# anyboby/Constrained-Model-Based-Policy-Optimization

Hardware: AMD Instinct MI355X
Metric: imagined env-steps/sec (ensemble rollout) + CPO update ms (higher is better)
Workload: dtype f32; 1 GPU; AntSafe-v2 imagined rollout: E=7 x (37->512->512->60) swish ensemble, 5 elites, 3+3 critics 128x128, tanh policy 128x128, B=100000 branches/GPU, maxroll 35 (34 steps), fixed-horizon mode, reset->sample*->finish_all_paths->get(); rollout_mode=schedule, branches_per_gpu=100000, branches_total=100000, horizon=34, task=AntSafe-v2

## Files before the change

constrained-model-based-policy-optimization_amd/csrc/fakeenv_post.hip:

```cpp
#include "common.h"

#include <math.h>

#include <type_traits>

namespace {

typedef float f32x2 __attribute__((ext_vector_type(2)));

constexpr int kThreads = 256;
constexpr int kRows = 8;
constexpr int kEMaxRt = 8;
constexpr int kEMax = kEMaxRt;

struct PostArgs {
  int task, ensemble, obs_dim, act_dim, out_dim;
  int learned_cost;
  const float *mean, *var;
  int ld_rows;
  const float *obs, *act;
  const int32_t *elite, *row_idx, *n_rows_dev;
  int n_rows;
  float *next_obs, *rew;
  uint8_t *term;
// ... 7 lines not shown
  const float *xi;
};
struct PostArgsRulesNoise : PostArgsRules {
  const float *xi;
};
template <bool RULES, bool NOISE>
using PostArgsBase = std::conditional_t<NOISE, std::conditional_t<RULES, PostArgsRulesNoise, PostArgsNoise>,
                                        std::conditional_t<RULES, PostArgsRules, PostArgs>>;
template <bool RULES, bool NOISE>
struct PostArgsDis : PostArgsBase<RULES, NOISE> {
  float kappa_rew, kappa_cost;
  float *rew_var, *cost_var;
};
template <bool RULES, bool NOISE, bool DIS = false>
using PostArgsT = std::conditional_t<DIS, PostArgsDis<RULES, NOISE>, PostArgsBase<RULES, NOISE>>;

__device__ __forceinline__ float clip_np(float x, float lo, float hi) { return x < lo ? lo : (x > hi ? hi : x); }

#define POST_WAVES 5
template <int EC, bool RULES = false, bool NOISE = false, bool DIS = false>
__global__ __launch_bounds__(kThreads) __attribute__((amdgpu_waves_per_eu(POST_WAVES, POST_WAVES))) void fakeenv_post_kernel(const PostArgsT<RULES, NOISE, DIS> p) {
  extern __shared__ float sm[];
  const int D = p.obs_dim;
  float *s_dkl = sm;
  float *s_var = s_dkl + kRows * D;
  float *s_next = s_var + kRows * D;
  int *s_row = reinterpret_cast<int *>(s_next + kRows * D);

  const int tid = threadIdx.x;
  const int n_rows = p.n_rows_dev ? *p.n_rows_dev : p.n_rows;
  const int row0 = blockIdx.x * kRows;
  if (row0 >= n_rows) return;
  if (tid < kRows) {
    const int r = row0 + tid;
    s_row[tid] = (r < n_rows) ? (p.row_idx ? p.row_idx[r] : r) : -1;
  }
  __syncthreads();

  const int E = EC > 0 ? EC : p.ensemble;
  constexpr int kEMax = EC > 0 ? EC : ::kEMaxRt;
  const size_t mstride = (size_t)p.ld_rows * p.out_dim;
  for (int i = tid; i < kRows * D; i += kThreads) {
    const int b = i / D, d = i - b * D;
    const int r = s_row[b];
    if (r < 0) continue;
    float mu[kEMax], ls[kEMax], vr[kEMax];
    bool fast = EC > 0;
    const size_t base = (size_t)r * p.out_dim + d;
    float v0s[kEMax];
#pragma unroll
// ... 95 lines not shown
              const float q = __fmul_rn(num, rden[c]);
              float pre = __fmul_rn(0.5f, __fsub_rn(q, 1.0f));
              pre = __fsub_rn(__fadd_rn(pre, ls[c]), ls[a]);
              pre = clip_np(pre, 0.0f, 1e10f);
              acc = __fadd_rn(acc, pre);
            }
          }
          if (!isfinite(vr[a]) || !isfinite(mu[a])) acc = __fadd_rn(acc, __builtin_nanf(""));
        }
      }
    }
    s_dkl[i] = acc / ((float)(E * (E - 1)) + 1e-10f);
    const float nx = __fadd_rn(mean_me, obs_rd);
    s_next[i] = nx;
    p.next_obs[(size_t)r * D + d] = nx;
    if (p.ep_var) p.ep_var[(size_t)r * D + d] = s_var[i];
  }
  __syncthreads();

  if (tid < 8 * kRows) {
    const int rw = tid >> 3, k = tid & 7;
    const int r = s_row[rw];
    const float *nx = s_next + rw * D;
    [[maybe_unused]] float xr = 0.0f, xc = 0.0f;
    [[maybe_unused]] int me_k = 0;
    if constexpr (DIS) {
      if (r >= 0) {
        me_k = p.elite[r];
        if (k < E) {
          const size_t o = k * mstride + (size_t)r * p.out_dim + D;
// ... 99 lines not shown
      const bool notdone = __fmul_rn(gate, zrot) >= -0.7f;
      done = notdone ? 0 : 1;
      const float obj = (fabsf(nx[D - 1]) > 3.2f) ? 1.0f : 0.0f;
      cost = fminf(fmaxf((float)done + obj, 0.0f), 1.0f);
    } else if (p.task == CMBPO_TASK_HCS) {
      const float xdist = __fmul_rn(nx[D - 1], 10.0f);
      cost = (fabsf(xdist) < 2.0f) ? 1.0f : 0.0f;
    }
    if constexpr (DIS) {
      if (p.learned_cost) cost = p.kappa_cost > 0.0f ? __fadd_rn(cost_me, __fmul_rn(p.kappa_cost, sqrtf(cost_var))) : cost_me;
    } else {
      if (p.learned_cost) cost = p.mean[me * mstride + (size_t)r * p.out_dim + D + 1];
    }
    p.term[r] = done;
    p.cost[r] = cost;
  }
}

template <bool RULES, bool NOISE, bool DIS = false>
void launch_post(int ensemble, dim3 grid, size_t lds, hipStream_t stream, const PostArgsT<RULES, NOISE, DIS> &a) {
  if (ensemble == 7) hipLaunchKernelGGL((fakeenv_post_kernel<7, RULES, NOISE, DIS>), grid, dim3(kThreads), lds, stream, a);
  else if (ensemble == 5) hipLaunchKernelGGL((fakeenv_post_kernel<5, RULES, NOISE, DIS>), grid, dim3(kThreads), lds, stream, a);
  else hipLaunchKernelGGL((fakeenv_post_kernel<0, RULES, NOISE, DIS>), grid, dim3(kThreads), lds, stream, a);
}

struct DisExtra {
  float kappa_rew, kappa_cost;
  float *rew_var, *cost_var;
};
template <bool RULES, bool NOISE>
void launch_post_dis(int ensemble, dim3 grid, size_t lds, hipStream_t stream, const PostArgsBase<RULES, NOISE> &a, const DisExtra &dis) {
  PostArgsDis<RULES, NOISE> ad{};
  static_cast<PostArgsBase<RULES, NOISE> &>(ad) = a;
  ad.kappa_rew = dis.kappa_rew; ad.kappa_cost = dis.kappa_cost; ad.rew_var = dis.rew_var; ad.cost_var = dis.cost_var;
  launch_post<RULES, NOISE, true>(ensemble, grid, lds, stream, ad);
}

int post_impl(const char *who, int task, int ensemble, int obs_dim, int act_dim, const float *d_mean, const float *d_var, int ld_rows,
              const float *d_obs, const float *d_act, const int32_t *d_elite, const int32_t *d_row_idx, const int32_t *d_n_rows,
              int n_rows, float *d_next_obs, float *d_rew, uint8_t *d_term, float *d_cost, float *d_dkl_path, float *d_ep_var_mean,
              float *d_ep_var, const float *d_xi, void *stream, const DisExtra *dis = nullptr) {
  const int learned_cost = (task & CMBPO_TASK_LEARNED_COST) ? 1 : 0;
  const int task_arg = task;
  task &= ~CMBPO_TASK_LEARNED_COST;
  const bool user = task >= CMBPO_TASK_USER_BASE && task < CMBPO_TASK_USER_BASE + CMBPO_TASK_USER_SLOTS;
  CMBPO_REQUIRE((task >= CMBPO_TASK_DEFAULT && task <= CMBPO_TASK_ANTSAFE) || user, "%s: bad task %d", who, task_arg);
  CMBPO_REQUIRE(ensemble >= 2 && ensemble <= kEMax, "%s: ensemble %d not in [2, %d]", who, ensemble, kEMax);
  CMBPO_REQUIRE(obs_dim >= 1 && obs_dim <= 512 && act_dim >= 0, "%s: bad dims", who);
  if (task == CMBPO_TASK_ANTSAFE)
    CMBPO_REQUIRE(obs_dim >= 5, "%s: AntSafe rules need obs_dim >= 5", who);
  PostArgsRules ar{};
  if (user)
    if (int rc = cmbpo_internal_task_rules_resolve(who, task_arg, obs_dim, act_dim, d_act != nullptr, &ar.rules)) return rc;
  CMBPO_REQUIRE(d_mean && d_var && d_obs && d_elite && d_next_obs && d_rew && d_term && d_cost &&
                    d_dkl_path && d_ep_var_mean,
                "%s: NULL buffer", who);
// ... 12 lines not shown
  a.out_dim = obs_dim + 1 + learned_cost;
  a.learned_cost = learned_cost;
  a.mean = d_mean; a.var = d_var; a.ld_rows = ld_rows; a.obs = d_obs; a.act = d_act;
  a.elite = d_elite; a.row_idx = d_row_idx; a.n_rows_dev = d_n_rows; a.n_rows = n_rows;
  a.next_obs = d_next_obs; a.rew = d_rew; a.term = d_term; a.cost = d_cost;
  a.dkl_path = d_dkl_path; a.ep_var_mean = d_ep_var_mean; a.ep_var = d_ep_var;
  const size_t lds = (size_t)3 * kRows * obs_dim * sizeof(float) + kRows * sizeof(int);
  const dim3 grid(cmbpo_ceil_div(n_rows, kRows));
  hipStream_t s = (hipStream_t)stream;
  if (user) static_cast<PostArgs &>(ar) = a;
  if (d_xi != nullptr) {
    if (user) {
      PostArgsRulesNoise an{};
      static_cast<PostArgsRules &>(an) = ar;
      an.xi = d_xi;
      if (dis) launch_post_dis<true, true>(ensemble, grid, lds, s, an, *dis);
      else launch_post<true, true>(ensemble, grid, lds, s, an);
    } else {
      PostArgsNoise an{};
      static_cast<PostArgs &>(an) = a;
      an.xi = d_xi;
      if (dis) launch_post_dis<false, true>(ensemble, grid, lds, s, an, *dis);
      else launch_post<false, true>(ensemble, grid, lds, s, an);
    }
  } else if (dis) {
    if (user) launch_post_dis<true, false>(ensemble, grid, lds, s, ar, *dis);
    else launch_post_dis<false, false>(ensemble, grid, lds, s, a, *dis);
  } else if (user) launch_post<true, false>(ensemble, grid, lds, s, ar);
  else launch_post<false, false>(ensemble, grid, lds, s, a);
  CMBPO_HIP_CHECK(hipGetLastError());
  return CMBPO_OK;
}

}

extern "C" int cmbpo_fakeenv_post(int task, int ensemble, int obs_dim, int act_dim,
                                  const float *d_mean, const float *d_var, int ld_rows,
                                  const float *d_obs, const float *d_act, const int32_t *d_elite,
                                  const int32_t *d_row_idx, const int32_t *d_n_rows, int n_rows,
                                  float *d_next_obs, float *d_rew, uint8_t *d_term, float *d_cost,
                                  float *d_dkl_path, float *d_ep_var_mean, float *d_ep_var,
                                  void *stream) {
  return post_impl("cmbpo_fakeenv_post", task, ensemble, obs_dim, act_dim, d_mean, d_var, ld_rows, d_obs, d_act, d_elite, d_row_idx,
                   d_n_rows, n_rows, d_next_obs, d_rew, d_term, d_cost, d_dkl_path, d_ep_var_mean, d_ep_var, nullptr, stream);
// ... 14 lines not shown
}

extern "C" int cmbpo_fakeenv_post_disagreement(int task, int ensemble, int obs_dim, int act_dim,
                                               const float *d_mean, const float *d_var, int ld_rows,
                                               const float *d_obs, const float *d_act, const int32_t *d_elite,
                                               const int32_t *d_row_idx, const int32_t *d_n_rows, int n_rows,
                                               float *d_next_obs, float *d_rew, uint8_t *d_term, float *d_cost,
                                               float *d_dkl_path, float *d_ep_var_mean, float *d_ep_var,
                                               const float *d_xi, float kappa_rew, float kappa_cost,
                                               float *d_rew_var, float *d_cost_var, void *stream) {
  const DisExtra dis{kappa_rew, kappa_cost, d_rew_var, d_cost_var};
  return post_impl("cmbpo_fakeenv_post_disagreement", task, ensemble, obs_dim, act_dim, d_mean, d_var, ld_rows, d_obs, d_act, d_elite,
                   d_row_idx, d_n_rows, n_rows, d_next_obs, d_rew, d_term, d_cost, d_dkl_path, d_ep_var_mean, d_ep_var, d_xi, stream,
                   &dis);
}
```

constrained-model-based-policy-optimization_amd/csrc/rollout_internal.h:

```cpp
#pragma once
#include "common.h"

int cmbpo_internal_book_post_mirror(const cmbpo_rollout_t *r, int n_alive, uint32_t *d_host_out, uint32_t seq, int spec, int min_alive,
                                    double stop_total, void *stream);
int cmbpo_internal_scalars_mirror(const cmbpo_rollout_t *r, uint32_t *d_host_out, uint32_t seq, void *stream);
int cmbpo_internal_book_pre(const cmbpo_rollout_t *r, int n_alive, int spec, int with_vec, void *stream);
int cmbpo_internal_store_nostats(const cmbpo_rollout_t *r, void *stream);
int cmbpo_internal_finish_post_fold(const cmbpo_rollout_t *r, void *stream);
int cmbpo_internal_spec_words(const cmbpo_rollout_t *r, int begin, void *stream);
int cmbpo_internal_disagreement_lookup(const cmbpo_rollout_t *r, cmbpo_disagreement_t *out);
```

constrained-model-based-policy-optimization_amd/csrc/rollout_state.hip:

```cpp
#include "common.h"
#include "rollout_internal.h"
#include <type_traits>

#include <math.h>

#include <mutex>
#include <unordered_map>

namespace {

constexpr int kScanThreads = 1024;

__device__ __forceinline__ int wave_incl_scan(int v, int lane) {
#pragma unroll
  for (int o = 1; o < 64; o <<= 1) {
    const int t = __shfl_up(v, o, 64);
    if (lane >= o) v += t;
  }
  return v;
}

__device__ __forceinline__ int block_excl_scan(int v, int *sm, int *total) {
  const int lane = threadIdx.x & 63, w = threadIdx.x >> 6, nw = (blockDim.x + 63) >> 6;
  const int inc = wave_incl_scan(v, lane);
// ... 232 lines not shown
    }
    const float cdelta = __fsub_rn(__fadd_rn(c, __fmul_rn(cg32, cvnext)), cv);
    y = __dadd_rn(delta, __dmul_rn(gl, y));
    cy = __dadd_rn((double)cdelta, __dmul_rn(cgl, cy));
    const float adv = (float)y, cadv = (float)cy;
    r.adv_buf[o] = adv;
    r.ret_buf[o] = __fadd_rn(adv, v);
    r.cadv_buf[o] = cadv;
    r.cret_buf[o] = __fadd_rn(cadv, cv);
    vnext = v;
    cvnext = cv;
  }
  r.alive[b] = 0;
}

__device__ __forceinline__ void store_stats_body(const cmbpo_rollout_t &r, const cmbpo_disagreement_t &dg);
__global__ __launch_bounds__(256) void finish_kernel(const cmbpo_rollout_t r, int mode, int fold_stats, const cmbpo_iv_gae_t iv,
                                                  const cmbpo_disagreement_t dg) {
  if (fold_stats && blockIdx.x == 0) store_stats_body(r, dg);
  const int i = blockIdx.x * blockDim.x + threadIdx.x;
  const int n = r.iscal[CMBPO_I_N_ALIVE];
  if (i >= n) return;
  const int b = r.alive_idx[i];
  float lv, lcv;
  bool zero_boot = false;
  if (mode == 0) {
    const uint8_t code = r.fin_code[b];
    if (!code) return;
    lv = r.v_t[b];
    lcv = r.vc_t[b];
    if (code == 2) {
      lv = 0.0f;
      zero_boot = true;
    }
// ... 86 lines not shown
  float *vdst[4] = {r.obs_buf, r.act_buf, r.mu_buf, r.ls_buf};
  const int vdim[4] = {D, A, A, A};
#pragma unroll
  for (int f = 0; f < 4; ++f) {
    const int dim = vdim[f];
    const float inv = 1.0f / (float)dim;
    for (int e = tid; e < rows_here * dim; e += 256) {
      const int k = (int)(((float)e + 0.5f) * inv);
      const int d = e - k * dim;
      const int b = s_slot[k];
      if (b >= 0) vdst[f][((size_t)r.ptr * B + b) * dim + d] = vsrc[f][(size_t)b * dim + d];
    }
  }
}

__device__ __forceinline__ void store_stats_body(const cmbpo_rollout_t &r, const cmbpo_disagreement_t &dg) {
  __shared__ double sm_d[16];
  const int n = r.iscal[CMBPO_I_N_ALIVE];
  const int n_wg = (n + kStoreRows - 1) / kStoreRows;
  double t[8] = {0, 0, 0, 0, 0, 0, 0, 0};
  for (int w = threadIdx.x; w < n_wg; w += 256) {
    const double *src = r.store_part + (size_t)w * 8;
#pragma unroll
    for (int k = 0; k < 6; ++k) t[k] += src[k];
    t[6] = fmax(t[6], src[6]);
    t[7] = fmax(t[7], src[7]);
  }
  double s[8];
#pragma unroll
  for (int k = 0; k < 6; ++k) s[k] = block_sum(t[k], sm_d);
  s[6] = block_max(t[6], sm_d);
  s[7] = block_max(t[7], sm_d);
  if (threadIdx.x == 0 && s[0] > 0.0) {
    const double cnt = s[0];
    const double dkl_mean = r.dscal[CMBPO_D_DKL_SUM_T] / (double)n;
    r.iscal[CMBPO_I_N_STORED] += (int)cnt;
    r.iscal[CMBPO_I_SIZE] += (int)cnt;
    r.dscal[CMBPO_D_TOTAL_SAMPLES] += cnt;
    r.dscal[CMBPO_D_TOTAL_COST] += s[1];
    r.dscal[CMBPO_D_TOTAL_REW] += s[2];
    r.dscal[CMBPO_D_SUM_PATH_RET] += s[2];
// ... 8 lines not shown
  if (dg.part != nullptr) {
    double u0 = 0.0, u1 = 0.0;
    for (int w = threadIdx.x; w < n_wg; w += 256) {
      u0 += dg.part[2 * (size_t)w];
      u1 += dg.part[2 * (size_t)w + 1];
    }
    u0 = block_sum(u0, sm_d);
    u1 = block_sum(u1, sm_d);
    if (threadIdx.x == 0 && s[0] > 0.0) {
      r.dscal[CMBPO_D_TOTAL_REW_VAR] += u0;
      r.dscal[CMBPO_D_TOTAL_COST_VAR] += u1;
    }
  }
}

__global__ __launch_bounds__(256) void store_stats_kernel(const cmbpo_rollout_t r, const cmbpo_disagreement_t dg) { store_stats_body(r, dg); }

constexpr int kBookMax = 1024;

__global__ __launch_bounds__(kScanThreads) void book_pre_kernel(const cmbpo_rollout_t r, int spec, const cmbpo_iv_gae_t iv,
                                                             const cmbpo_disagreement_t dg) {
  __shared__ int sm_i[17];
  __shared__ double sm_d[16];
  __shared__ double sm_m[8 * 16];
  __shared__ int s_unc;
  const int tid = threadIdx.x;
  if (spec && r.iscal[CMBPO_I_HALT]) return;
  const int n = r.iscal[CMBPO_I_N_ALIVE];
  {
    double c = 0.0, d = 0.0;
    for (int i = tid; i < n; i += kScanThreads) {
// ... 785 lines not shown
  CMBPO_REQUIRE(r->cur_obs && r->act_t && r->logp_t && r->mu_t && r->ls_t && r->v_t && r->vc_t && r->rew_t && r->cost_t && r->dkl_t &&
                    r->epv_t && r->obs_buf && r->act_buf && r->mu_buf && r->ls_buf && r->rew_buf && r->val_buf && r->cost_buf &&
                    r->cval_buf && r->logp_buf && r->store_part,
                "cmbpo_rollout_store: NULL array");
  hipLaunchKernelGGL(store_kernel, dim3(cmbpo_ceil_div(r->B, kStoreRows)), dim3(256), 0, (hipStream_t)stream, *r, iv_lookup(r),
                     dg_lookup(r));
  CMBPO_HIP_CHECK(hipGetLastError());
  return CMBPO_OK;
}
int cmbpo_internal_finish_post_fold(const cmbpo_rollout_t *r, void *stream) {
  if (int rc = check_rollout(r, "cmbpo_rollout_finish")) return rc;
  CMBPO_REQUIRE(r->v_n && r->vc_n && r->term_t && r->rew_buf && r->val_buf && r->cost_buf && r->cval_buf && r->adv_buf && r->ret_buf &&
                    r->cadv_buf && r->cret_buf && r->store_part,
                "cmbpo_rollout_finish (POST): NULL array");
  hipLaunchKernelGGL(finish_kernel, dim3(cmbpo_ceil_div(r->B, 256)), dim3(256), 0, (hipStream_t)stream, *r, 1, 1, iv_lookup(r), dg_lookup(r));
  CMBPO_HIP_CHECK(hipGetLastError());
  return CMBPO_OK;
}

extern "C" int cmbpo_rollout_book_pre_max_rows(void) { return kBookMax; }

extern "C" int cmbpo_rollout_book_pre(const cmbpo_rollout_t *r, int n_alive, void *stream) {
  if (int rc = check_rollout(r, "cmbpo_rollout_book_pre")) return rc;
  CMBPO_REQUIRE(n_alive >= 0 && n_alive <= kBookMax, "cmbpo_rollout_book_pre: %d alive rows, at most %d", n_alive, kBookMax);
  CMBPO_REQUIRE(!r->use_host_budget, "cmbpo_rollout_book_pre: the cross-shard budget exchange uses the separate kernels");
  CMBPO_REQUIRE(r->ptr < r->T, "cmbpo_rollout_book_pre: buffer full (ptr %d == T)", r->ptr);
  CMBPO_REQUIRE(r->dkl_t && r->dkl_acc && r->cur_obs && r->act_t && r->logp_t && r->mu_t && r->ls_t && r->v_t && r->vc_t &&
                    r->rew_t && r->cost_t && r->epv_t,
                "cmbpo_rollout_book_pre: NULL step array");
  CMBPO_REQUIRE(r->obs_buf && r->act_buf && r->mu_buf && r->ls_buf && r->rew_buf && r->val_buf && r->cost_buf && r->cval_buf &&
// ... 200 lines not shown
```

constrained-model-based-policy-optimization_amd/csrc/rollout_step.hip:

```cpp
#include "common.h"
#include "ens_mlp_internal.h"
#include "rollout_internal.h"

#include <string.h>
#include <time.h>

#include <atomic>
#include <mutex>

struct Ahead {
  bool on = false;
  int min_alive = 0;
  double stop_total = 0.0;
};

static int step_impl(const cmbpo_rollout_t *r, int n_alive, cmbpo_mlp_t *policy, cmbpo_mlp_t *model, cmbpo_mlp_t *v,
                     cmbpo_mlp_t *vc, int task, int ensemble, const float *d_eps, const int32_t *d_elite, float *d_mean,
                     float *d_var, bool policy_ready, const float *d_eps_next, bool *next_ready, uint32_t *d_mirror, uint32_t seq,
                     const Ahead &ahead, const float *d_xi, void *stream) {
  CMBPO_REQUIRE(r && policy && model && v && vc && d_eps && d_elite && d_mean && d_var, "cmbpo_rollout_step: NULL argument");
  CMBPO_REQUIRE(n_alive >= 1 && n_alive <= r->B, "cmbpo_rollout_step: n_alive %d not in [1, B=%d]", n_alive, r->B);
  CMBPO_REQUIRE(model->out_dim == r->obs_dim + 1 + ((task & CMBPO_TASK_LEARNED_COST) ? 1 : 0),
                "cmbpo_rollout_step: model out_dim %d does not match obs_dim %d + 1 (+ 1 with CMBPO_TASK_LEARNED_COST), task 0x%x",
                model->out_dim, r->obs_dim, task);
  if ((task & ~CMBPO_TASK_LEARNED_COST) >= CMBPO_TASK_USER_BASE)
    if (int rc0 = cmbpo_internal_task_rules_resolve("cmbpo_rollout_step", task, r->obs_dim, r->act_dim, r->act_t != nullptr, nullptr)) return rc0;
  auto w = [](const float *p) { return const_cast<float *>(p); };
  int rc;
  *next_ready = false;
  const int32_t *d_n = ahead.on ? r->iscal + CMBPO_I_N_EFF : nullptr;
  if (ahead.on)
    CMBPO_REQUIRE(n_alive <= cmbpo_rollout_book_pre_max_rows() && !r->use_host_budget && d_mirror && cmbpo_critic_pair_supported(v, vc),
                  "cmbpo_rollout_run: look-ahead needs the small-batch step");
  if (!policy_ready &&
      (rc = cmbpo_policy_forward(policy, r->cur_obs, r->obs_dim, d_eps, r->alive_idx, d_n, n_alive, w(r->act_t), w(r->logp_t),
                                 w(r->mu_t), w(r->ls_t), stream)))
    return rc;
  if ((rc = cmbpo_ens_forward(model, r->cur_obs, r->obs_dim, r->act_t, r->act_dim, r->alive_idx, d_n, n_alive, r->B,
                              d_mean, d_var, stream)))
    return rc;
  cmbpo_disagreement_t dg;
  if (cmbpo_internal_disagreement_lookup(r, &dg)) {
    if ((rc = cmbpo_fakeenv_post_disagreement(task, ensemble, r->obs_dim, r->act_dim, d_mean, d_var, r->B, r->cur_obs, r->act_t, d_elite,
                                              r->alive_idx, d_n, n_alive, w(r->next_obs), w(r->rew_t), const_cast<uint8_t *>(r->term_t),
                                              w(r->cost_t), w(r->dkl_t), w(r->epv_t), nullptr, d_xi, dg.kappa_rew, dg.kappa_cost,
                                              dg.rew_var_t, dg.cost_var_t, stream)))
      return rc;
  } else
  if ((rc = cmbpo_fakeenv_post_noise(task, ensemble, r->obs_dim, r->act_dim, d_mean, d_var, r->B, r->cur_obs, r->act_t, d_elite,
                                     r->alive_idx, d_n, n_alive, w(r->next_obs), w(r->rew_t), const_cast<uint8_t *>(r->term_t),
                                     w(r->cost_t), w(r->dkl_t), w(r->epv_t), nullptr, d_xi, stream)))
    return rc;
  const bool small = ahead.on || (n_alive <= cmbpo_rollout_book_pre_max_rows() && !r->use_host_budget);
  const bool vec_rides = small && cmbpo_critic_pair_supported(v, vc) && n_alive < kCriticBigMin;
  if (small) {
    if ((rc = cmbpo_internal_book_pre(r, n_alive, ahead.on ? 1 : 0, vec_rides ? 0 : 1, stream))) return rc;
  } else {
    const bool fold_late = !r->use_host_budget;
    if ((rc = cmbpo_rollout_decide(r, stream))) return rc;
    if (r->uncertainty_mode || r->max_samples != 0 || r->use_host_budget)
      if ((rc = cmbpo_rollout_finish(r, 0, stream))) return rc;
    if ((rc = fold_late ? cmbpo_internal_store_nostats(r, stream) : cmbpo_rollout_store(r, stream))) return rc;
  }
  if (cmbpo_critic_pair_supported(v, vc)) {
    const bool ride = d_eps_next != nullptr && n_alive < kCriticBigMin &&
                      cmbpo_internal_critic_pair_can_ride(v, vc, policy);
    CmbpoStoreVec sv{};
    if (vec_rides) {
      const float *src[4] = {r->cur_obs, r->act_t, r->mu_t, r->ls_t};
      float *dst[4] = {r->obs_buf, r->act_buf, r->mu_buf, r->ls_buf};
      const int dim[4] = {r->obs_dim, r->act_dim, r->act_dim, r->act_dim};
      for (int f = 0; f < 4; ++f) { sv.src[f] = src[f]; sv.dst[f] = dst[f]; sv.dim[f] = dim[f]; }
// ... 4 lines not shown
                                              ride ? policy : nullptr, d_eps_next, w(r->act_t), w(r->logp_t), w(r->mu_t), w(r->ls_t),
                                              stream, vec_rides ? &sv : nullptr)))
      return rc;
    *next_ready = ride;
  } else {
    if ((rc = cmbpo_ens_predict_mean(v, r->next_obs, r->obs_dim, r->alive_idx, nullptr, n_alive, w(r->v_n), stream))) return rc;
    if ((rc = cmbpo_ens_predict_mean(vc, r->next_obs, r->obs_dim, r->alive_idx, nullptr, n_alive, w(r->vc_n), stream))) return rc;
  }
  if (small) {
    if ((rc = d_mirror ? cmbpo_internal_book_post_mirror(r, n_alive, d_mirror, seq, ahead.on ? 1 : 0, ahead.min_alive, ahead.stop_total,
                                                         stream)
                       : cmbpo_rollout_book_post(r, n_alive, stream)))
      return rc;
    return 1;
  }
  return r->use_host_budget ? cmbpo_rollout_finish(r, 1, stream) : cmbpo_internal_finish_post_fold(r, stream);
}

extern "C" int cmbpo_rollout_step(const cmbpo_rollout_t *r, int n_alive, cmbpo_mlp_t *policy, cmbpo_mlp_t *model,
                                  cmbpo_mlp_t *v, cmbpo_mlp_t *vc, int task, int ensemble, const float *d_eps,
                                  const int32_t *d_elite, float *d_mean, float *d_var, void *stream) {
  bool unused = false;
  return step_impl(r, n_alive, policy, model, v, vc, task, ensemble, d_eps, d_elite, d_mean, d_var, false, nullptr, &unused, nullptr, 0u,
                   Ahead{}, r ? r->xi : nullptr, stream);
}

namespace {
constexpr int kMirrorSlots = 64, kMirrorDwords = 128, kMaxDevices = 64;
struct Mirror {
  uint32_t *h = nullptr, *d = nullptr;
  bool tried = false;
};
Mirror g_mirror[kMaxDevices];
std::mutex g_mirror_mu;
std::atomic<uint32_t> g_seq{0};

uint32_t next_seq() {
  uint32_t s = g_seq.fetch_add(1, std::memory_order_relaxed) + 1;
  return s ? s : g_seq.fetch_add(1, std::memory_order_relaxed) + 1;
// ... 59 lines not shown
    }
    { const float *t = r->cur_obs; r->cur_obs = r->next_obs; r->next_obs = t; }
    { const float *t = r->v_t; r->v_t = r->v_n; r->v_n = t; }
    { const float *t = r->vc_t; r->vc_t = r->vc_n; r->vc_n = t; }
    r->ptr += 1;
  };
  while (done < max_steps && n_alive > 0 && r->ptr < r->T) {
    Mirror &mir = mirror();
    if (mir.d && n_alive <= cmbpo_rollout_book_pre_max_rows() && cmbpo_critic_pair_supported(v, vc)) {
      Ahead ah;
      ah.on = true; ah.min_alive = min_alive; ah.stop_total = stop_total;
      if (int rc = cmbpo_internal_spec_words(r, 1, stream)) return rc;
      struct Pend { int slot; uint32_t seq; };
      auto enqueue = [&](int k, Pend &p) -> int {
        const float *eps_next = k + 1 < max_steps ? d_eps + (size_t)(k + 1) * eps_stride : nullptr;
        bool next_ready = false;
        p.slot = k % kMirrorSlots;
        p.seq = next_seq();
        const int rc = step_impl(r, n_alive, policy, model, v, vc, task, ensemble, d_eps + (size_t)k * eps_stride,
                                 d_elite + (size_t)k * elite_stride, d_mean, d_var, ready, eps_next, &next_ready,
                                 mir.d + (size_t)p.slot * kMirrorDwords, p.seq, ah, xi_at(k), stream);
        ready = next_ready;
        if (rc == 0) cmbpo_set_error("cmbpo_rollout_run: look-ahead step took the large-batch path");
        return rc == 1 ? CMBPO_OK : (rc == 0 ? CMBPO_EINVAL : rc);
      };
      Pend cur{}, nxt{};
      if (int rc = enqueue(done, cur)) return rc;
      bool halted = false;
      for (;;) {
        advance(true);
        const bool more = done + 1 < max_steps && r->ptr < r->T;
        if (more)
          if (int rc = enqueue(done + 1, nxt)) return rc;
        const uint32_t *h_slot = mir.h + (size_t)cur.slot * kMirrorDwords;
        if (int rc2 = wait_mirror(h_slot, cur.seq, (hipStream_t)stream)) return rc2;
        char *h = static_cast<char *>(h_scalars) + (size_t)done * 384;
        memcpy(h, h_slot, 384);
        const int32_t *isc = reinterpret_cast<const int32_t *>(h);
        n_alive = isc[CMBPO_I_N_ALIVE];
        halted = isc[CMBPO_I_HALT] != 0;
        ++done;
        if (halted || !more) break;
        cur = nxt;
      }
      if (halted)
        if (int rc = cmbpo_internal_spec_words(r, 0, stream)) return rc;
      break;
    }
    const float *eps_next = done + 1 < max_steps ? d_eps + (size_t)(done + 1) * eps_stride : nullptr;
    bool next_ready = false;
    const int slot = done % kMirrorSlots;
    const uint32_t seq = next_seq();
    uint32_t *d_slot = mir.d ? mir.d + (size_t)slot * kMirrorDwords : nullptr;
    int rc = step_impl(r, n_alive, policy, model, v, vc, task, ensemble, d_eps + (size_t)done * eps_stride,
                       d_elite + (size_t)done * elite_stride, d_mean, d_var, ready, eps_next, &next_ready, d_slot, seq, Ahead{},
                       xi_at(done), stream);
    ready = next_ready;
    if (rc != 0 && rc != 1) return rc;
    char *h = static_cast<char *>(h_scalars) + (size_t)done * 384;
    if (rc == 1 && d_slot != nullptr) {
      const uint32_t *h_slot = mir.h + (size_t)slot * kMirrorDwords;
      if (int rc2 = wait_mirror(h_slot, seq, (hipStream_t)stream)) return rc2;
      memcpy(h, h_slot, 384);
    } else if (d_slot != nullptr) {
      const uint32_t *h_slot = mir.h + (size_t)slot * kMirrorDwords;
      if (int rc2 = cmbpo_internal_scalars_mirror(r, d_slot, seq, stream)) return rc2;
      if (eps_next != nullptr && !ready && r->ptr + 1 < r->T) {
        auto w = [](const float *q) { return const_cast<float *>(q); };
        if (int rc2 = cmbpo_policy_forward(policy, r->next_obs, r->obs_dim, eps_next, r->alive_idx, nullptr, n_alive, w(r->act_t),
                                           w(r->logp_t), w(r->mu_t), w(r->ls_t), stream))
          return rc2;
        ready = true;
      }
      if (int rc2 = wait_mirror(h_slot, seq, (hipStream_t)stream)) return rc2;
      memcpy(h, h_slot, 384);
    } else if (int rc2 = cmbpo_rollout_read_scalars(r, h, stream)) {
      return rc2;
    }
    const int32_t *isc = reinterpret_cast<const int32_t *>(h);
    const double *dsc = reinterpret_cast<const double *>(h + 128);
    const int fin = isc[CMBPO_I_N_FIN_PRE] + isc[CMBPO_I_N_FIN_POST];
// ... 17 lines not shown
```

Before: 73.87 million imagined env-steps/s.

## Fuse buffer store into post kernel and fold finish/stats/mirror into two kernels

For large-batch fixed-horizon steps, the fakeenv post kernel now also writes obs/act/mu/ls/logp into the rollout buffers and resets per-step scalars. The separate decide/store/finish/stats/mirror launches are replaced by a finish_store kernel and a single-block fold_step kernel that also writes the host scalar mirror. This cuts kernel launches and redundant passes over per-branch data each step. In exchange it adds a specialized code path with a hoisted reduction that assumes B fits within a fixed block count, and correctness depends on the scalar resets matching the old decide logic.

Measured after the change: 74.25 million imagined env-steps/s (median of 6 runs). Within noise of the previous version (+0.5%).

```diff
diff --git a/constrained-model-based-policy-optimization_amd/csrc/fakeenv_post.hip b/constrained-model-based-policy-optimization_amd/csrc/fakeenv_post.hip
--- a/constrained-model-based-policy-optimization_amd/csrc/fakeenv_post.hip
+++ b/constrained-model-based-policy-optimization_amd/csrc/fakeenv_post.hip
@@ -1,4 +1,5 @@
 #include "common.h"
+#include "rollout_internal.h"
 
 #include <math.h>
 
@@ -45,12 +46,18 @@
 };
 template <bool RULES, bool NOISE, bool DIS = false>
 using PostArgsT = std::conditional_t<DIS, PostArgsDis<RULES, NOISE>, PostArgsBase<RULES, NOISE>>;
+template <bool RULES, bool NOISE, bool DIS>
+struct PostArgsStore : PostArgsT<RULES, NOISE, DIS> {
+  cmbpo_rollout_t r;
+};
+template <bool RULES, bool NOISE, bool DIS, bool STORE>
+using PostKernArgs = std::conditional_t<STORE, PostArgsStore<RULES, NOISE, DIS>, PostArgsT<RULES, NOISE, DIS>>;
 
 __device__ __forceinline__ float clip_np(float x, float lo, float hi) { return x < lo ? lo : (x > hi ? hi : x); }
 
 #define POST_WAVES 5
-template <int EC, bool RULES = false, bool NOISE = false, bool DIS = false>
-__global__ __launch_bounds__(kThreads) __attribute__((amdgpu_waves_per_eu(POST_WAVES, POST_WAVES))) void fakeenv_post_kernel(const PostArgsT<RULES, NOISE, DIS> p) {
+template <int EC, bool RULES = false, bool NOISE = false, bool DIS = false, bool STORE = false>
+__global__ __launch_bounds__(kThreads) __attribute__((amdgpu_waves_per_eu(POST_WAVES, POST_WAVES))) void fakeenv_post_kernel(const PostKernArgs<RULES, NOISE, DIS, STORE> p) {
   extern __shared__ float sm[];
   const int D = p.obs_dim;
   float *s_dkl = sm;
@@ -65,6 +72,19 @@
   if (tid < kRows) {
     const int r = row0 + tid;
     s_row[tid] = (r < n_rows) ? (p.row_idx ? p.row_idx[r] : r) : -1;
+    if constexpr (STORE) {
+      if (s_row[tid] >= 0) p.r.fin_code[s_row[tid]] = 0;
+      if (blockIdx.x == 0 && tid == 0) {
+        p.r.iscal[CMBPO_I_N_UNC] = 0;
+        p.r.iscal[CMBPO_I_N_STORED] = 0;
+        p.r.iscal[CMBPO_I_N_FIN_POST] = 0;
+        p.r.iscal[8] = p.r.iscal[CMBPO_I_N_ALIVE];
+        p.r.iscal[9] = 0;
+        p.r.iscal[10] = (int)p.r.dscal[CMBPO_D_TOTAL_SAMPLES];
+        p.r.iscal[11] = 0;
+        p.r.iscal[CMBPO_I_N_FIN_PRE] = 0;
+      }
+    }
   }
   __syncthreads();
 
@@ -190,6 +210,7 @@
     const float nx = __fadd_rn(mean_me, obs_rd);
     s_next[i] = nx;
     p.next_obs[(size_t)r * D + d] = nx;
+    if constexpr (STORE) p.r.obs_buf[((size_t)p.r.ptr * (size_t)p.r.B + r) * D + d] = obs_rd;
     if (p.ep_var) p.ep_var[(size_t)r * D + d] = s_var[i];
   }
   __syncthreads();
@@ -319,11 +340,40 @@
     }
     p.term[r] = done;
     p.cost[r] = cost;
+  } else if constexpr (STORE) {
+    const int A = p.r.act_dim;
+    const float *vsrc[3] = {p.r.act_t, p.r.mu_t, p.r.ls_t};
+    float *vdst[3] = {p.r.act_buf, p.r.mu_buf, p.r.ls_buf};
+    const size_t col = (size_t)p.r.ptr * (size_t)p.r.B;
+    if (tid - 8 * kRows < kRows && s_row[tid - 8 * kRows] >= 0) {
+      const int b = s_row[tid - 8 * kRows];
+      p.r.logp_buf[col + b] = p.r.logp_t[b];
+    }
+    for (int e = tid - 8 * kRows; e < kRows * A; e += kThreads - 8 * kRows) {
+      const int k = e / A, d = e - k * A;
+      const int b = s_row[k];
+      if (b < 0) continue;
+#pragma unroll
+      for (int f = 0; f < 3; ++f) vdst[f][(col + b) * A + d] = vsrc[f][(size_t)b * A + d];
+    }
   }
 }
 
+template <bool RULES, bool NOISE, bool DIS>
+void launch_post_store(int ensemble, dim3 grid, size_t lds, hipStream_t stream, const PostArgsT<RULES, NOISE, DIS> &a,
+                       const cmbpo_rollout_t *store) {
+  PostArgsStore<RULES, NOISE, DIS> as{};
+  static_cast<PostArgsT<RULES, NOISE, DIS> &>(as) = a;
+  as.r = *store;
+  if (ensemble == 7) hipLaunchKernelGGL((fakeenv_post_kernel<7, RULES, NOISE, DIS, true>), grid, dim3(kThreads), lds, stream, as);
+  else if (ensemble == 5) hipLaunchKernelGGL((fakeenv_post_kernel<5, RULES, NOISE, DIS, true>), grid, dim3(kThreads), lds, stream, as);
+  else hipLaunchKernelGGL((fakeenv_post_kernel<0, RULES, NOISE, DIS, true>), grid, dim3(kThreads), lds, stream, as);
+}
+
 template <bool RULES, bool NOISE, bool DIS = false>
-void launch_post(int ensemble, dim3 grid, size_t lds, hipStream_t stream, const PostArgsT<RULES, NOISE, DIS> &a) {
+void launch_post(int ensemble, dim3 grid, size_t lds, hipStream_t stream, const PostArgsT<RULES, NOISE, DIS> &a,
+                 const cmbpo_rollout_t *store) {
+  if (store != nullptr) return launch_post_store<RULES, NOISE, DIS>(ensemble, grid, lds, stream, a, store);
   if (ensemble == 7) hipLaunchKernelGGL((fakeenv_post_kernel<7, RULES, NOISE, DIS>), grid, dim3(kThreads), lds, stream, a);
   else if (ensemble == 5) hipLaunchKernelGGL((fakeenv_post_kernel<5, RULES, NOISE, DIS>), grid, dim3(kThreads), lds, stream, a);
   else hipLaunchKernelGGL((fakeenv_post_kernel<0, RULES, NOISE, DIS>), grid, dim3(kThreads), lds, stream, a);
@@ -334,17 +384,18 @@
   float *rew_var, *cost_var;
 };
 template <bool RULES, bool NOISE>
-void launch_post_dis(int ensemble, dim3 grid, size_t lds, hipStream_t stream, const PostArgsBase<RULES, NOISE> &a, const DisExtra &dis) {
+void launch_post_dis(int ensemble, dim3 grid, size_t lds, hipStream_t stream, const PostArgsBase<RULES, NOISE> &a, const DisExtra &dis,
+                     const cmbpo_rollout_t *store) {
   PostArgsDis<RULES, NOISE> ad{};
   static_cast<PostArgsBase<RULES, NOISE> &>(ad) = a;
   ad.kappa_rew = dis.kappa_rew; ad.kappa_cost = dis.kappa_cost; ad.rew_var = dis.rew_var; ad.cost_var = dis.cost_var;
-  launch_post<RULES, NOISE, true>(ensemble, grid, lds, stream, ad);
+  launch_post<RULES, NOISE, true>(ensemble, grid, lds, stream, ad, store);
 }
 
 int post_impl(const char *who, int task, int ensemble, int obs_dim, int act_dim, const float *d_mean, const float *d_var, int ld_rows,
               const float *d_obs, const float *d_act, const int32_t *d_elite, const int32_t *d_row_idx, const int32_t *d_n_rows,
               int n_rows, float *d_next_obs, float *d_rew, uint8_t *d_term, float *d_cost, float *d_dkl_path, float *d_ep_var_mean,
-              float *d_ep_var, const float *d_xi, void *stream, const DisExtra *dis = nullptr) {
+              float *d_ep_var, const float *d_xi, void *stream, const DisExtra *dis = nullptr, const cmbpo_rollout_t *store = nullptr) {
   const int learned_cost = (task & CMBPO_TASK_LEARNED_COST) ? 1 : 0;
   const int task_arg = task;
   task &= ~CMBPO_TASK_LEARNED_COST;
@@ -387,20 +438,20 @@
       PostArgsRulesNoise an{};
       static_cast<PostArgsRules &>(an) = ar;
       an.xi = d_xi;
-      if (dis) launch_post_dis<true, true>(ensemble, grid, lds, s, an, *dis);
-      else launch_post<true, true>(ensemble, grid, lds, s, an);
+      if (dis) launch_post_dis<true, true>(ensemble, grid, lds, s, an, *dis, store);
+      else launch_post<true, true>(ensemble, grid, lds, s, an, store);
     } else {
       PostArgsNoise an{};
       static_cast<PostArgs &>(an) = a;
       an.xi = d_xi;
-      if (dis) launch_post_dis<false, true>(ensemble, grid, lds, s, an, *dis);
-      else launch_post<false, true>(ensemble, grid, lds, s, an);
+      if (dis) launch_post_dis<false, true>(ensemble, grid, lds, s, an, *dis, store);
+      else launch_post<false, true>(ensemble, grid, lds, s, an, store);
     }
   } else if (dis) {
-    if (user) launch_post_dis<true, false>(ensemble, grid, lds, s, ar, *dis);
-    else launch_post_dis<false, false>(ensemble, grid, lds, s, a, *dis);
-  } else if (user) launch_post<true, false>(ensemble, grid, lds, s, ar);
-  else launch_post<false, false>(ensemble, grid, lds, s, a);
+    if (user) launch_post_dis<true, false>(ensemble, grid, lds, s, ar, *dis, store);
+    else launch_post_dis<false, false>(ensemble, grid, lds, s, a, *dis, store);
+  } else if (user) launch_post<true, false>(ensemble, grid, lds, s, ar, store);
+  else launch_post<false, false>(ensemble, grid, lds, s, a, store);
   CMBPO_HIP_CHECK(hipGetLastError());
   return CMBPO_OK;
 }
@@ -445,3 +496,20 @@
                    d_row_idx, d_n_rows, n_rows, d_next_obs, d_rew, d_term, d_cost, d_dkl_path, d_ep_var_mean, d_ep_var, d_xi, stream,
                    &dis);
 }
+
+int cmbpo_internal_fakeenv_post_store(const cmbpo_rollout_t *r, int task, int ensemble, const float *d_mean, const float *d_var,
+                                      const int32_t *d_elite, int n_alive, const float *d_xi, const cmbpo_disagreement_t *dg,
+                                      void *stream) {
+  const char *who = "cmbpo_rollout_step (post + store)";
+  CMBPO_REQUIRE(r && r->alive_idx && r->iscal && r->dscal && r->fin_code && r->act_t && r->mu_t && r->ls_t && r->logp_t && r->obs_buf &&
+                    r->act_buf && r->mu_buf && r->ls_buf && r->logp_buf,
+                "%s: NULL array", who);
+  CMBPO_REQUIRE(r->ptr >= 0 && r->ptr < r->T, "%s: buffer full (ptr %d, T %d)", who, r->ptr, r->T);
+  CMBPO_REQUIRE(n_alive >= 1 && n_alive <= r->B, "%s: n_alive %d not in [1, B=%d]", who, n_alive, r->B);
+  auto w = [](const float *q) { return const_cast<float *>(q); };
+  DisExtra dis{};
+  if (dg != nullptr) dis = DisExtra{dg->kappa_rew, dg->kappa_cost, dg->rew_var_t, dg->cost_var_t};
+  return post_impl(who, task, ensemble, r->obs_dim, r->act_dim, d_mean, d_var, r->B, r->cur_obs, r->act_t, d_elite, r->alive_idx,
+                           nullptr, n_alive, w(r->next_obs), w(r->rew_t), const_cast<uint8_t *>(r->term_t), w(r->cost_t), w(r->dkl_t),
+                           w(r->epv_t), nullptr, d_xi, stream, dg != nullptr ? &dis : nullptr, r);
+}
diff --git a/constrained-model-based-policy-optimization_amd/csrc/rollout_internal.h b/constrained-model-based-policy-optimization_amd/csrc/rollout_internal.h
--- a/constrained-model-based-policy-optimization_amd/csrc/rollout_internal.h
+++ b/constrained-model-based-policy-optimization_amd/csrc/rollout_internal.h
@@ -9,3 +9,8 @@
 int cmbpo_internal_finish_post_fold(const cmbpo_rollout_t *r, void *stream);
 int cmbpo_internal_spec_words(const cmbpo_rollout_t *r, int begin, void *stream);
 int cmbpo_internal_disagreement_lookup(const cmbpo_rollout_t *r, cmbpo_disagreement_t *out);
+int cmbpo_internal_fakeenv_post_store(const cmbpo_rollout_t *r, int task, int ensemble, const float *d_mean, const float *d_var,
+                                      const int32_t *d_elite, int n_alive, const float *d_xi, const cmbpo_disagreement_t *dg,
+                                      void *stream);
+bool cmbpo_internal_fused_store_supported(const cmbpo_rollout_t *r);
+int cmbpo_internal_finish_store(const cmbpo_rollout_t *r, uint32_t *d_host_out, uint32_t seq, void *stream);
diff --git a/constrained-model-based-policy-optimization_amd/csrc/rollout_state.hip b/constrained-model-based-policy-optimization_amd/csrc/rollout_state.hip
--- a/constrained-model-based-policy-optimization_amd/csrc/rollout_state.hip
+++ b/constrained-model-based-policy-optimization_amd/csrc/rollout_state.hip
@@ -270,10 +270,11 @@
   r.alive[b] = 0;
 }
 
+template <bool HOIST = false>
 __device__ __forceinline__ void store_stats_body(const cmbpo_rollout_t &r, const cmbpo_disagreement_t &dg);
 __global__ __launch_bounds__(256) void finish_kernel(const cmbpo_rollout_t r, int mode, int fold_stats, const cmbpo_iv_gae_t iv,
                                                   const cmbpo_disagreement_t dg) {
-  if (fold_stats && blockIdx.x == 0) store_stats_body(r, dg);
+  if (fold_stats && blockIdx.x == 0) store_stats_body<false>(r, dg);
   const int i = blockIdx.x * blockDim.x + threadIdx.x;
   const int n = r.iscal[CMBPO_I_N_ALIVE];
   if (i >= n) return;
@@ -390,17 +391,38 @@
   }
 }
 
+template <bool HOIST>
 __device__ __forceinline__ void store_stats_body(const cmbpo_rollout_t &r, const cmbpo_disagreement_t &dg) {
   __shared__ double sm_d[16];
   const int n = r.iscal[CMBPO_I_N_ALIVE];
   const int n_wg = (n + kStoreRows - 1) / kStoreRows;
   double t[8] = {0, 0, 0, 0, 0, 0, 0, 0};
-  for (int w = threadIdx.x; w < n_wg; w += 256) {
-    const double *src = r.store_part + (size_t)w * 8;
-#pragma unroll
-    for (int k = 0; k < 6; ++k) t[k] += src[k];
-    t[6] = fmax(t[6], src[6]);
-    t[7] = fmax(t[7], src[7]);
+  if constexpr (HOIST) {
+    double v[8][8];
+#pragma unroll
+    for (int j = 0; j < 8; ++j) {
+      const int w = threadIdx.x + 256 * j;
+      const double *src = r.store_part + (size_t)(w < n_wg ? w : 0) * 8;
+#pragma unroll
+      for (int k = 0; k < 8; ++k) v[j][k] = src[k];
+    }
+#pragma unroll
+    for (int j = 0; j < 8; ++j) {
+      if ((int)threadIdx.x + 256 * j < n_wg) {
+#pragma unroll
+        for (int k = 0; k < 6; ++k) t[k] += v[j][k];
+        t[6] = fmax(t[6], v[j][6]);
+        t[7] = fmax(t[7], v[j][7]);
+      }
+    }
+  } else {
+    for (int w = threadIdx.x; w < n_wg; w += 256) {
+      const double *src = r.store_part + (size_t)w * 8;
+#pragma unroll
+      for (int k = 0; k < 6; ++k) t[k] += src[k];
+      t[6] = fmax(t[6], src[6]);
+      t[7] = fmax(t[7], src[7]);
+    }
   }
   double s[8];
 #pragma unroll
@@ -439,7 +461,124 @@
   }
 }
 
-__global__ __launch_bounds__(256) void store_stats_kernel(const cmbpo_rollout_t r, const cmbpo_disagreement_t dg) { store_stats_body(r, dg); }
+__global__ __launch_bounds__(256) void store_stats_kernel(const cmbpo_rollout_t r, const cmbpo_disagreement_t dg) { store_stats_body<false>(r, dg); }
+
+constexpr int kDecideBlocksMax = 512;
+
+__device__ __forceinline__ void fold_step_body(const cmbpo_rollout_t &r, const cmbpo_disagreement_t &dg, int n_blocks) {
+  __shared__ double sm_w[16];
+  const int tid = threadIdx.x;
+  const int n = r.iscal[CMBPO_I_N_ALIVE];
+  const int n_live = (n + 255) / 256;
+#pragma unroll
+  for (int g = 0; g < 4; ++g) {
+    const int w = g * 256 + tid;
+    double d = 0.0;
+    if (w < n_live) d += r.store_part[(size_t)w * 32];
+    d = wave_sum(d);
+    if ((tid & 63) == 0) sm_w[g * 4 + (tid >> 6)] = d;
+  }
+  __syncthreads();
+  if (tid < 64) {
+    double t = tid < 16 ? sm_w[tid] : 0.0;
+    t = wave_sum(t);
+    if (tid == 0) r.dscal[CMBPO_D_DKL_SUM_T] = t;
+  }
+  __syncthreads();
+  for (int w = tid; w < n_live; w += 256) r.store_part[(size_t)w * 32] = (double)min(kStoreRows, n - w * 256);
+  const int n_tiles = (n + kStoreRows - 1) / kStoreRows;
+  for (int k = 8 * n_tiles + tid; k < 2 * n_blocks; k += 256) r.store_part[k] = 0.0;
+  __syncthreads();
+  store_stats_body<true>(r, dg);
+}
+
+__global__ __launch_bounds__(256) void finish_store_kernel(const cmbpo_rollout_t r, const cmbpo_iv_gae_t iv, const cmbpo_disagreement_t dg) {
+  __shared__ double sm_d[16];
+  const int n = r.iscal[CMBPO_I_N_ALIVE];
+  const int tid = threadIdx.x;
+  if ((int)blockIdx.x * 256 >= n) return;
+  const int i = blockIdx.x * 256 + tid;
+  const int tile = blockIdx.x * 4 + (tid >> 6);
+  const size_t B = (size_t)r.B;
+  const int D = r.obs_dim;
+  const int b = i < n ? r.alive_idx[i] : -1;
+  double a_cnt = 0, a_cost = 0, a_rew = 0, a_v = 0, a_vc = 0, a_epv = 0, a_maxdkl = 0, a_maxret = 0;
+  double dsum = 0.0;
+  if (b >= 0) {
+    const size_t col = (size_t)r.ptr * B + b;
+    const float rw = r.rew_t[b], c = r.cost_t[b], v = r.v_t[b], vc = r.vc_t[b];
+    const float epv = r.epv_t[b], dk = r.dkl_t[b];
+    r.rew_buf[col] = rw;
+    r.val_buf[col] = v;
+    r.cost_buf[col] = c;
+    r.cval_buf[col] = vc;
+    r.len[b] = r.ptr + 1;
+    const double pr = r.path_ret[b] + (double)rw;
+    r.path_ret[b] = pr;
+    r.path_cost[b] += (double)c;
+    const double pv = r.path_dyn_var[b] + (double)epv;
+    r.path_dyn_var[b] = pv;
+    if (iv.cumvar_buf != nullptr) iv.cumvar_buf[col] = pv;
+    r.dkl_acc[b] += (double)dk;
+    a_cnt = 1.0; a_cost = c; a_rew = rw; a_v = v; a_vc = vc;
+    a_epv = (double)epv * D;
+    a_maxdkl = (double)dk;
+    a_maxret = pr;
+    dsum += (double)dk;
+  }
+  const bool tile_live = tile * kStoreRows < n;
+  if (dg.part != nullptr) {
+    double a_rv = 0, a_cv = 0;
+    if (b >= 0) {
+      a_rv = (double)dg.rew_var_t[b];
+      a_cv = (double)dg.cost_var_t[b];
+      dg.path_rew_var[b] += a_rv;
+      dg.path_cost_var[b] += a_cv;
+    }
+    const double w0 = wave_sum(a_rv), w1 = wave_sum(a_cv);
+    if ((tid & 63) == 0 && tile_live) {
+      dg.part[2 * (size_t)tile] = w0;
+      dg.part[2 * (size_t)tile + 1] = w1;
+    }
+  }
+  const double v0 = wave_sum(a_cnt), v1 = wave_sum(a_cost), v2 = wave_sum(a_rew), v3 = wave_sum(a_v);
+  const double v4 = wave_sum(a_vc), v5 = wave_sum(a_epv), v6 = wave_max(a_maxdkl), v7 = wave_max(a_maxret);
+  const double dblk = block_sum(dsum, sm_d);
+  if ((tid & 63) == 0 && tile_live) {
+    double *dst = r.store_part + (size_t)tile * 8;
+    dst[0] = tid == 0 ? dblk : v0; dst[1] = v1; dst[2] = v2; dst[3] = v3; dst[4] = v4; dst[5] = v5; dst[6] = v6; dst[7] = v7;
+  }
+  if (b < 0) return;
+  float lv;
+  bool zero_boot = false;
+  const bool horizon = (r.ptr + 1 >= r.max_path_length - 1);
+  if (horizon) {
+    lv = r.v_n[b];
+  } else if (r.term_t[b]) {
+    lv = 0.0f;
+    zero_boot = true;
+  } else {
+    return;
+  }
+  atomicAdd(&r.iscal[CMBPO_I_N_FIN_POST], 1);
+  gae_finish_path(r, iv, b, lv, r.vc_n[b], zero_boot);
+}
+
+__global__ __launch_bounds__(256) void fold_step_kernel(const cmbpo_rollout_t r, const cmbpo_disagreement_t dg, int n_blocks,
+                                                     uint32_t *host_out, uint32_t seq) {
+  fold_step_body(r, dg, n_blocks);
+  if (host_out != nullptr && threadIdx.x == 0) {
+    const uint4 *src = reinterpret_cast<const uint4 *>(r.iscal);
+    uint4 *dst = reinterpret_cast<uint4 *>(host_out);
+    uint4 q[24];
+#pragma unroll
+    for (int k = 0; k < 24; ++k) q[k] = src[k];
+#pragma unroll
+    for (int k = 0; k < 24; ++k) dst[k] = q[k];
+    __threadfence_system();
+    *reinterpret_cast<volatile uint32_t *>(host_out + 96) = seq;
+  }
+}
 
 constexpr int kBookMax = 1024;
 
@@ -1255,6 +1394,26 @@
                     r->cadv_buf && r->cret_buf && r->store_part,
                 "cmbpo_rollout_finish (POST): NULL array");
   hipLaunchKernelGGL(finish_kernel, dim3(cmbpo_ceil_div(r->B, 256)), dim3(256), 0, (hipStream_t)stream, *r, 1, 1, iv_lookup(r), dg_lookup(r));
+  CMBPO_HIP_CHECK(hipGetLastError());
+  return CMBPO_OK;
+}
+
+bool cmbpo_internal_fused_store_supported(const cmbpo_rollout_t *r) {
+  return !r->uncertainty_mode && r->max_samples == 0 && !r->use_host_budget && r->B <= kDecideBlocksMax * 256;
+}
+int cmbpo_internal_finish_store(const cmbpo_rollout_t *r, uint32_t *d_host_out, uint32_t seq, void *stream) {
+  if (int rc = check_rollout(r, "cmbpo_rollout_step (store + finish)")) return rc;
+  CMBPO_REQUIRE(cmbpo_internal_fused_store_supported(r) && r->ptr < r->T, "cmbpo_rollout_step (store + finish): bad state");
+  CMBPO_REQUIRE(r->v_t && r->vc_t && r->rew_t && r->cost_t && r->dkl_t && r->epv_t && r->dkl_acc && r->path_ret &&
+                    r->path_cost && r->path_dyn_var && r->rew_buf && r->val_buf && r->cost_buf && r->cval_buf &&
+                    r->store_part && r->v_n && r->vc_n && r->term_t && r->adv_buf && r->ret_buf && r->cadv_buf && r->cret_buf,
+                "cmbpo_rollout_step (store + finish): NULL array");
+  CMBPO_REQUIRE(d_host_out == nullptr || reinterpret_cast<const char *>(r->dscal) == reinterpret_cast<const char *>(r->iscal) + 128,
+                "scalars mirror: iscal[32] and dscal[32] must be one 384-byte block");
+  const cmbpo_disagreement_t dg = dg_lookup(r);
+  const int n_blocks = cmbpo_ceil_div(r->B, 256);
+  hipLaunchKernelGGL(finish_store_kernel, dim3(n_blocks), dim3(256), 0, (hipStream_t)stream, *r, iv_lookup(r), dg);
+  hipLaunchKernelGGL(fold_step_kernel, dim3(1), dim3(256), 0, (hipStream_t)stream, *r, dg, n_blocks, d_host_out, seq);
   CMBPO_HIP_CHECK(hipGetLastError());
   return CMBPO_OK;
 }
diff --git a/constrained-model-based-policy-optimization_amd/csrc/rollout_step.hip b/constrained-model-based-policy-optimization_amd/csrc/rollout_step.hip
--- a/constrained-model-based-policy-optimization_amd/csrc/rollout_step.hip
+++ b/constrained-model-based-policy-optimization_amd/csrc/rollout_step.hip
@@ -17,7 +17,7 @@
 static int step_impl(const cmbpo_rollout_t *r, int n_alive, cmbpo_mlp_t *policy, cmbpo_mlp_t *model, cmbpo_mlp_t *v,
                      cmbpo_mlp_t *vc, int task, int ensemble, const float *d_eps, const int32_t *d_elite, float *d_mean,
                      float *d_var, bool policy_ready, const float *d_eps_next, bool *next_ready, uint32_t *d_mirror, uint32_t seq,
-                     const Ahead &ahead, const float *d_xi, void *stream) {
+                     const Ahead &ahead, const float *d_xi, bool *mirrored, void *stream) {
   CMBPO_REQUIRE(r && policy && model && v && vc && d_eps && d_elite && d_mean && d_var, "cmbpo_rollout_step: NULL argument");
   CMBPO_REQUIRE(n_alive >= 1 && n_alive <= r->B, "cmbpo_rollout_step: n_alive %d not in [1, B=%d]", n_alive, r->B);
   CMBPO_REQUIRE(model->out_dim == r->obs_dim + 1 + ((task & CMBPO_TASK_LEARNED_COST) ? 1 : 0),
@@ -28,6 +28,7 @@
   auto w = [](const float *p) { return const_cast<float *>(p); };
   int rc;
   *next_ready = false;
+  *mirrored = false;
   const int32_t *d_n = ahead.on ? r->iscal + CMBPO_I_N_EFF : nullptr;
   if (ahead.on)
     CMBPO_REQUIRE(n_alive <= cmbpo_rollout_book_pre_max_rows() && !r->use_host_budget && d_mirror && cmbpo_critic_pair_supported(v, vc),
@@ -39,8 +40,14 @@
   if ((rc = cmbpo_ens_forward(model, r->cur_obs, r->obs_dim, r->act_t, r->act_dim, r->alive_idx, d_n, n_alive, r->B,
                               d_mean, d_var, stream)))
     return rc;
+  const bool small = ahead.on || (n_alive <= cmbpo_rollout_book_pre_max_rows() && !r->use_host_budget);
+  const bool fused = !small && cmbpo_internal_fused_store_supported(r);
   cmbpo_disagreement_t dg;
-  if (cmbpo_internal_disagreement_lookup(r, &dg)) {
+  const bool has_dg = cmbpo_internal_disagreement_lookup(r, &dg) != 0;
+  if (fused) {
+    if ((rc = cmbpo_internal_fakeenv_post_store(r, task, ensemble, d_mean, d_var, d_elite, n_alive, d_xi, has_dg ? &dg : nullptr, stream)))
+      return rc;
+  } else if (has_dg) {
     if ((rc = cmbpo_fakeenv_post_disagreement(task, ensemble, r->obs_dim, r->act_dim, d_mean, d_var, r->B, r->cur_obs, r->act_t, d_elite,
                                               r->alive_idx, d_n, n_alive, w(r->next_obs), w(r->rew_t), const_cast<uint8_t *>(r->term_t),
                                               w(r->cost_t), w(r->dkl_t), w(r->epv_t), nullptr, d_xi, dg.kappa_rew, dg.kappa_cost,
@@ -51,11 +58,10 @@
                                      r->alive_idx, d_n, n_alive, w(r->next_obs), w(r->rew_t), const_cast<uint8_t *>(r->term_t),
                                      w(r->cost_t), w(r->dkl_t), w(r->epv_t), nullptr, d_xi, stream)))
     return rc;
-  const bool small = ahead.on || (n_alive <= cmbpo_rollout_book_pre_max_rows() && !r->use_host_budget);
   const bool vec_rides = small && cmbpo_critic_pair_supported(v, vc) && n_alive < kCriticBigMin;
   if (small) {
     if ((rc = cmbpo_internal_book_pre(r, n_alive, ahead.on ? 1 : 0, vec_rides ? 0 : 1, stream))) return rc;
-  } else {
+  } else if (!fused) {
     const bool fold_late = !r->use_host_budget;
     if ((rc = cmbpo_rollout_decide(r, stream))) return rc;
     if (r->uncertainty_mode || r->max_samples != 0 || r->use_host_budget)
@@ -90,15 +96,20 @@
       return rc;
     return 1;
   }
+  if (fused) {
+    if ((rc = cmbpo_internal_finish_store(r, d_mirror, seq, stream))) return rc;
+    *mirrored = d_mirror != nullptr;
+    return 0;
+  }
   return r->use_host_budget ? cmbpo_rollout_finish(r, 1, stream) : cmbpo_internal_finish_post_fold(r, stream);
 }
 
 extern "C" int cmbpo_rollout_step(const cmbpo_rollout_t *r, int n_alive, cmbpo_mlp_t *policy, cmbpo_mlp_t *model,
                                   cmbpo_mlp_t *v, cmbpo_mlp_t *vc, int task, int ensemble, const float *d_eps,
                                   const int32_t *d_elite, float *d_mean, float *d_var, void *stream) {
-  bool unused = false;
+  bool unused = false, unused2 = false;
   return step_impl(r, n_alive, policy, model, v, vc, task, ensemble, d_eps, d_elite, d_mean, d_var, false, nullptr, &unused, nullptr, 0u,
-                   Ahead{}, r ? r->xi : nullptr, stream);
+                   Ahead{}, r ? r->xi : nullptr, &unused2, stream);
 }
 
 namespace {
@@ -188,12 +199,12 @@
       struct Pend { int slot; uint32_t seq; };
       auto enqueue = [&](int k, Pend &p) -> int {
         const float *eps_next = k + 1 < max_steps ? d_eps + (size_t)(k + 1) * eps_stride : nullptr;
-        bool next_ready = false;
+        bool next_ready = false, mirrored = false;
         p.slot = k % kMirrorSlots;
         p.seq = next_seq();
         const int rc = step_impl(r, n_alive, policy, model, v, vc, task, ensemble, d_eps + (size_t)k * eps_stride,
                                  d_elite + (size_t)k * elite_stride, d_mean, d_var, ready, eps_next, &next_ready,
-                                 mir.d + (size_t)p.slot * kMirrorDwords, p.seq, ah, xi_at(k), stream);
+                                 mir.d + (size_t)p.slot * kMirrorDwords, p.seq, ah, xi_at(k), &mirrored, stream);
         ready = next_ready;
         if (rc == 0) cmbpo_set_error("cmbpo_rollout_run: look-ahead step took the large-batch path");
         return rc == 1 ? CMBPO_OK : (rc == 0 ? CMBPO_EINVAL : rc);
@@ -222,13 +233,13 @@
       break;
     }
     const float *eps_next = done + 1 < max_steps ? d_eps + (size_t)(done + 1) * eps_stride : nullptr;
-    bool next_ready = false;
+    bool next_ready = false, mirrored = false;
     const int slot = done % kMirrorSlots;
     const uint32_t seq = next_seq();
     uint32_t *d_slot = mir.d ? mir.d + (size_t)slot * kMirrorDwords : nullptr;
     int rc = step_impl(r, n_alive, policy, model, v, vc, task, ensemble, d_eps + (size_t)done * eps_stride,
                        d_elite + (size_t)done * elite_stride, d_mean, d_var, ready, eps_next, &next_ready, d_slot, seq, Ahead{},
-                       xi_at(done), stream);
+                       xi_at(done), &mirrored, stream);
     ready = next_ready;
     if (rc != 0 && rc != 1) return rc;
     char *h = static_cast<char *>(h_scalars) + (size_t)done * 384;
@@ -238,7 +249,8 @@
       memcpy(h, h_slot, 384);
     } else if (d_slot != nullptr) {
       const uint32_t *h_slot = mir.h + (size_t)slot * kMirrorDwords;
-      if (int rc2 = cmbpo_internal_scalars_mirror(r, d_slot, seq, stream)) return rc2;
+      if (!mirrored)
+        if (int rc2 = cmbpo_internal_scalars_mirror(r, d_slot, seq, stream)) return rc2;
       if (eps_next != nullptr && !ready && r->ptr + 1 < r->T) {
         auto w = [](const float *q) { return const_cast<float *>(q); };
         if (int rc2 = cmbpo_policy_forward(policy, r->next_obs, r->obs_dim, eps_next, r->alive_idx, nullptr, n_alive, w(r->act_t),
```
